# crockwell/rel_pose

Hardware: AMD Instinct MI355X
Metric: image-pairs/sec fwd+bwd @384x384, 1/2/4/8 MI355X; R,t err vs ref (higher is better)
Workload: dtype f32; 1 GPU; train.py step (ViTEss fwd + geodesic loss + bwd + grad all-reduce + clip + Adam), synthetic 384x384 pairs; scope=full, pairs_per_gpu=64, global_batch_pairs=64, parallelism=dp1, finite=True, gemm_operand_precision=exact fp32 MFMA, launch=eager

## Files before the change

__graft_entry__.py:

```python
import os
import subprocess
import sys

ROOT = os.path.dirname(os.path.abspath(__file__))
if ROOT not in sys.path:
    sys.path.insert(0, ROOT)


def build():
    import torch
    from rel_pose_amd import _build
    force = os.environ.get("RP_FORCE_BUILD", "" if torch.cuda.is_available() else "1") == "1"
    _build.build(force=force, verbose=True)
    from rel_pose_amd import _lib
    lib = _lib.load()
    assert lib.rp_abi_version() == _lib.ABI_VERSION and lib.rp_target_arch() == b"gfx950"
    assert lib.rp_abi_export_count() == _lib.ABI_EXPORTS == len(_lib.EXPORTS)
    assert _lib.load_readout().rp_readout_abi_version() == _lib.READOUT_ABI_VERSION
    assert _lib.load_eightpoint().rp_eightpoint_abi_version() == _lib.EIGHTPOINT_ABI_VERSION
    assert _lib.load_refine().rp_refine_abi_version() == _lib.REFINE_ABI_VERSION
    assert _lib.load_consensus().rp_consensus_abi_version() == _lib.CONSENSUS_ABI_VERSION
    assert _lib.load_submatch().rp_submatch_abi_version() == _lib.SUBMATCH_ABI_VERSION
    assert _lib.load_fivepoint().rp_fivepoint_abi_version() == _lib.FIVEPOINT_ABI_VERSION
    assert _lib.load_homography().rp_homography_abi_version() == _lib.HOMOGRAPHY_ABI_VERSION
    assert _lib.load_triangulate().rp_triangulate_abi_version() == _lib.TRIANGULATE_ABI_VERSION
    import rel_pose_amd.model
    import oracle.relpose_oracle
    print("build ok:", _lib.lib_path(), _build.READOUT_LIB, _build.EIGHTPOINT_LIB, _build.REFINE_LIB, _build.CONSENSUS_LIB, _build.SUBMATCH_LIB,
          _build.FIVEPOINT_LIB, _build.HOMOGRAPHY_LIB, _build.TRIANGULATE_LIB)


def smoke():
    import types

    import torch

    from oracle import relpose_oracle as O
    from rel_pose_amd import _lib
    from rel_pose_amd.model import ViTEss
    assert torch.cuda.is_available(), "smoke() needs cuda:0"
    _lib.load()
    torch.cuda.set_device(0)
    args = types.SimpleNamespace(noess="", pool_size=60, fc_hidden_size=512, fusion_transformer=True,
                                 transformer_depth=6, cross_features=False, use_single_softmax=False,
                                 no_pos_encoding=False, l1_pos_encoding=False)
    shapes = dict(O.vit_param_shapes())
    shapes.update(O.cnn_param_shapes())
    sd32, sd64 = O.make_state(shapes, torch.float32), O.make_state(shapes, torch.float64)
    model = ViTEss(args)
    model.load_state_dict(sd32)
    model = model.cuda().train()
    tok = O.synthetic_tokens(2)
    Gs = torch.tensor([0, 0, 0, 0, 0, 0, 1.0]).repeat(1, 2, 1)
    intr = torch.tensor([[30.0, 26.0, 12.0, 11.0]]).repeat(1, 2, 1)
    fmap = tok.permute(0, 2, 1).contiguous().view(2, 192, 24, 24).cuda().requires_grad_(True)
    out = model.forward_tokens(fmap, Gs.cuda(), intr.cuda())
    out[:, 1].square().sum().backward()
    t64 = tok.double().requires_grad_(True)
    ref = O.vit_ess_from_tokens(sd64, t64, Gs.double(), intr.double())
    ref[:, 1].square().sum().backward()
    t_err, q_err, ang = O.pose_errors(out.detach().cpu(), ref.detach())
    g_err = O.rel_err(fmap.grad.view(2, 192, 576).permute(0, 2, 1).cpu(), t64.grad)
    print("smoke: t_err=%.2e q_err=%.2e angle=%.2e rad, token-grad rel err=%.2e" % (t_err, q_err, ang, g_err))
    assert max(t_err, q_err) < 1e-4 and g_err < 2e-5
    print("smoke ok (HIP path vs CPU oracle)")


if __name__ == "__main__":
    build()
    if len(sys.argv) > 1 and sys.argv[1] == "smoke":
        smoke()
```

rel_pose_amd/_build.py:

```python
import os
import subprocess
import sys

HERE = os.path.dirname(os.path.abspath(__file__))
CSRC = os.path.join(HERE, "csrc")
LIB = os.path.join(HERE, "librelpose_hip.so")
SOURCES = ["gemm.hip", "gemm_dma.hip", "rowwise.hip", "attention.hip", "attention_bf16.hip", "dw192_bf16.hip", "dw192_f32.hip", "dw192_split3.hip", "dx_lnbwd_bf16.hip", "emm.hip", "emm_bf16.hip", "batchnorm.hip", "se3loss.hip", "geom.hip", "augment.hip", "mlp_fused.hip", "linear_rows.hip", "conv_stem.hip", "conv_stem_bf16.hip", "conv_stem_wgrad_bf16.hip", "conv_stem_wgrad_f32.hip", "conv3x3_bf16.hip", "conv3x3_wgrad_bf16.hip", "conv3x3_wgrad_f32.hip", "conv3x3_f32.hip", "conv3x3_c128_f32.hip"]
READOUT_CSRC = os.path.join(HERE, "csrc_readout")
READOUT_LIB = os.path.join(HERE, "librelpose_readout.so")
READOUT_SOURCES = ["emm_readout.hip"]
EIGHTPOINT_CSRC = os.path.join(HERE, "csrc_eightpoint")
EIGHTPOINT_LIB = os.path.join(HERE, "librelpose_eightpoint.so")
EIGHTPOINT_SOURCES = ["eight_point.hip"]
REFINE_CSRC = os.path.join(HERE, "csrc_refine")
REFINE_LIB = os.path.join(HERE, "librelpose_refine.so")
REFINE_SOURCES = ["refine_pose.hip"]
CONSENSUS_CSRC = os.path.join(HERE, "csrc_consensus")
CONSENSUS_LIB = os.path.join(HERE, "librelpose_consensus.so")
CONSENSUS_SOURCES = ["consensus.hip"]
SUBMATCH_CSRC = os.path.join(HERE, "csrc_submatch")
SUBMATCH_LIB = os.path.join(HERE, "librelpose_submatch.so")
SUBMATCH_SOURCES = ["submatch.hip"]
FIVEPOINT_CSRC = os.path.join(HERE, "csrc_fivepoint")
FIVEPOINT_LIB = os.path.join(HERE, "librelpose_fivepoint.so")
FIVEPOINT_SOURCES = ["five_point.hip"]
HOMOGRAPHY_CSRC = os.path.join(HERE, "csrc_homography")
HOMOGRAPHY_LIB = os.path.join(HERE, "librelpose_homography.so")
HOMOGRAPHY_SOURCES = ["homography.hip"]
TRIANGULATE_CSRC = os.path.join(HERE, "csrc_triangulate")
TRIANGULATE_LIB = os.path.join(HERE, "librelpose_triangulate.so")
TRIANGULATE_SOURCES = ["triangulate.hip"]
ARCH = "gfx950"


def _hipcc():
    for c in (os.environ.get("HIPCC"), "/opt/rocm/bin/hipcc"):
        if c and os.path.exists(c):
            return c
    return "hipcc"


def _stale(lib, csrc, sources, headers):
    if not os.path.exists(lib):
        return True
    t = os.path.getmtime(lib)
    return any(os.path.getmtime(d) > t for d in [os.path.join(csrc, s) for s in sources] + headers)


def needs_build():
    return _stale(LIB, CSRC, SOURCES, _headers())


def readout_needs_build():
    return _stale(READOUT_LIB, READOUT_CSRC, READOUT_SOURCES, _readout_headers())


def eightpoint_needs_build():
    return _stale(EIGHTPOINT_LIB, EIGHTPOINT_CSRC, EIGHTPOINT_SOURCES, _eightpoint_headers())


def refine_needs_build():
    return _stale(REFINE_LIB, REFINE_CSRC, REFINE_SOURCES, _refine_headers())


def consensus_needs_build():
    return _stale(CONSENSUS_LIB, CONSENSUS_CSRC, CONSENSUS_SOURCES, _consensus_headers())


def submatch_needs_build():
    return _stale(SUBMATCH_LIB, SUBMATCH_CSRC, SUBMATCH_SOURCES, _submatch_headers())


def fivepoint_needs_build():
    return _stale(FIVEPOINT_LIB, FIVEPOINT_CSRC, FIVEPOINT_SOURCES, _fivepoint_headers())


def homography_needs_build():
    return _stale(HOMOGRAPHY_LIB, HOMOGRAPHY_CSRC, HOMOGRAPHY_SOURCES, _homography_headers())


def triangulate_needs_build():
    return _stale(TRIANGULATE_LIB, TRIANGULATE_CSRC, TRIANGULATE_SOURCES, _triangulate_headers())


def build(force=False, verbose=True):
    import fcntl
    with open(os.path.join(HERE, ".build.lock"), "w") as lock:
        fcntl.flock(lock, fcntl.LOCK_EX)
        try:
            if force or needs_build():
                _build_locked(verbose, force, LIB, CSRC, SOURCES, _headers())
            if force or readout_needs_build():
                _build_locked(verbose, force, READOUT_LIB, READOUT_CSRC, READOUT_SOURCES, _readout_headers())
            if force or eightpoint_needs_build():
                _build_locked(verbose, force, EIGHTPOINT_LIB, EIGHTPOINT_CSRC, EIGHTPOINT_SOURCES, _eightpoint_headers())
            if force or refine_needs_build():
                _build_locked(verbose, force, REFINE_LIB, REFINE_CSRC, REFINE_SOURCES, _refine_headers())
            if force or consensus_needs_build():
                _build_locked(verbose, force, CONSENSUS_LIB, CONSENSUS_CSRC, CONSENSUS_SOURCES, _consensus_headers())
            if force or submatch_needs_build():
                _build_locked(verbose, force, SUBMATCH_LIB, SUBMATCH_CSRC, SUBMATCH_SOURCES, _submatch_headers())
            if force or fivepoint_needs_build():
                _build_locked(verbose, force, FIVEPOINT_LIB, FIVEPOINT_CSRC, FIVEPOINT_SOURCES, _fivepoint_headers())
            if force or homography_needs_build():
                _build_locked(verbose, force, HOMOGRAPHY_LIB, HOMOGRAPHY_CSRC, HOMOGRAPHY_SOURCES, _homography_headers())
            if force or triangulate_needs_build():
                _build_locked(verbose, force, TRIANGULATE_LIB, TRIANGULATE_CSRC, TRIANGULATE_SOURCES, _triangulate_headers())
            return LIB
        finally:
            fcntl.flock(lock, fcntl.LOCK_UN)


def _headers():
    return [os.path.join(CSRC, h) for h in sorted(os.listdir(CSRC)) if h.endswith(".h")] + \
           [os.path.join(os.path.dirname(HERE), "include", "relpose_hip.h")]


def _readout_headers():
    return _headers() + [os.path.join(os.path.dirname(HERE), "include", "relpose_readout.h")]


def _eightpoint_headers():
    return _headers() + [os.path.join(os.path.dirname(HERE), "include", "relpose_eightpoint.h")]


def _refine_headers():
    return _headers() + [os.path.join(os.path.dirname(HERE), "include", "relpose_refine.h")]


def _consensus_headers():
    return _headers() + [os.path.join(os.path.dirname(HERE), "include", "relpose_consensus.h")]


def _submatch_headers():
    return _headers() + [os.path.join(os.path.dirname(HERE), "include", "relpose_submatch.h")]


def _fivepoint_headers():
    return _headers() + [os.path.join(os.path.dirname(HERE), "include", "relpose_fivepoint.h")]


def _homography_headers():
    return _headers() + [os.path.join(os.path.dirname(HERE), "include", "relpose_homography.h")]


def _triangulate_headers():
    return _headers() + [os.path.join(os.path.dirname(HERE), "include", "relpose_triangulate.h")]


def _build_locked(verbose, force, lib, csrc, sources, headers):
    cc = _hipcc()
    objs = []
    procs = []
    hdr_t = max(os.path.getmtime(h) for h in headers)
    for s in sources:
        o = os.path.join(csrc, s.replace(".hip", ".o"))
        objs.append(o)
        if not force and os.path.exists(o) and os.path.getmtime(o) > max(hdr_t, os.path.getmtime(os.path.join(csrc, s))):
            continue
        cmd = [cc, "--offload-arch=" + ARCH, "-O3", "-std=c++17", "-fPIC", "-c", os.path.join(csrc, s), "-o", o]
        if verbose:
            print(" ".join(cmd), flush=True)
        procs.append((s, subprocess.Popen(cmd, stdout=subprocess.PIPE, stderr=subprocess.STDOUT)))
    for s, p in procs:
        out, _ = p.communicate()
        if p.returncode != 0:
            sys.stderr.write(out.decode())
            raise RuntimeError("hipcc failed on " + s)
    tmp = lib + ".tmp.%d" % os.getpid()
    cmd = [cc, "--offload-arch=" + ARCH, "-shared", "-fPIC", "-o", tmp] + objs
    if verbose:
        print(" ".join(cmd), flush=True)
    subprocess.check_call(cmd)
    os.replace(tmp, lib)
    return lib


if __name__ == "__main__":
    build(force="--force" in sys.argv)
```

rel_pose_amd/_lib.py:

```python
import ctypes
import keyword
import os
import re
from ctypes import POINTER, Structure, c_char_p, c_float, c_int, c_longlong, c_size_t, c_void_p

import torch

from . import _build

_LIB = None
HEADER = os.path.join(os.path.dirname(os.path.dirname(os.path.abspath(__file__))), "include", "relpose_hip.h")

_SCALARS = {"int": c_int, "float": c_float, "long long": c_longlong, "size_t": c_size_t}
_POINTEES = ("void", "float", "double", "int", "unsigned char")
_DEFINE = re.compile(r"#\s*define\s+(RP_\w+)\s+(-?\d+|\(-?\d+\))")
_DECL = re.compile(r"(const\s+)?(unsigned\s+char|long\s+long|\w+)\s*(\*?)\s*([A-Za-z_]\w*(?:\s*,\s*[A-Za-z_]\w*)*)?")
_ITEM = re.compile(r"\s*(?:typedef\s+struct\s+(\w+)\s*\{([^{}]*);\s*\}\s*(\w+)\s*;"
                   r"|([\w\s*]+?)\b(rp_\w+)\s*\(([^()]*)\)\s*;"
                   r'|extern\s+"C"\s*\{|\})')


def _declaration(text, structs, header="relpose_hip.h"):
    m = _DECL.fullmatch(text.strip())
    if not m:
# ... 54 lines not shown
with open(HEADER) as _f:
    _CONSTS, _STRUCTS, _PROTOTYPES, _STATUS = _header_contract(_f.read())
ABI_VERSION, ABI_EXPORTS = _CONSTS["RP_ABI_VERSION"], _CONSTS["RP_ABI_EXPORTS"]
RP_COLSUM_MAX, RP_SPLITK_MAX, RP_TRANSPOSE_MAX = _CONSTS["RP_COLSUM_MAX"], _CONSTS["RP_SPLITK_MAX"], _CONSTS["RP_TRANSPOSE_MAX"]
_ERROR_TEXT = {"RP_EBADSHAPE": "bad shape", "RP_EALIGN": "misaligned pointer/stride", "RP_EWORKSPACE": "workspace too small",
               "RP_EUNSUPPORTED": "unsupported"}
RP_ERRORS = {code: _ERROR_TEXT[name] for name, code in _CONSTS.items() if name.startswith("RP_E")}
RpGemm, RpColsumTask, RpBnMask, RpSplitkTask, RpTransposeTask = (
    _STRUCTS[n] for n in ("RpGemm", "RpColsumTask", "RpBnMask", "RpSplitkTask", "RpTransposeTask"))
EXPORTS = tuple(_PROTOTYPES)
DECLARED = set(EXPORTS)


_READOUT_LIB = None
READOUT_HEADER = os.path.join(os.path.dirname(HEADER), "relpose_readout.h")
with open(READOUT_HEADER) as _f:
    _READOUT_CONSTS, _, _READOUT_PROTOTYPES, _READOUT_STATUS = _header_contract(_f.read(), "relpose_readout.h")
READOUT_ABI_VERSION = _READOUT_CONSTS["RP_READOUT_ABI_VERSION"]
READOUT_EXPORTS = tuple(_READOUT_PROTOTYPES)


_EIGHTPOINT_LIB = None
EIGHTPOINT_HEADER = os.path.join(os.path.dirname(HEADER), "relpose_eightpoint.h")
with open(EIGHTPOINT_HEADER) as _f:
    _EIGHTPOINT_CONSTS, _, _EIGHTPOINT_PROTOTYPES, _EIGHTPOINT_STATUS = _header_contract(_f.read(), "relpose_eightpoint.h")
EIGHTPOINT_ABI_VERSION = _EIGHTPOINT_CONSTS["RP_EIGHTPOINT_ABI_VERSION"]
EIGHTPOINT_MAX_P, EIGHTPOINT_MAX_ITERS = _EIGHTPOINT_CONSTS["RP_EIGHTPOINT_MAX_P"], _EIGHTPOINT_CONSTS["RP_EIGHTPOINT_MAX_ITERS"]
EIGHTPOINT_EXPORTS = tuple(_EIGHTPOINT_PROTOTYPES)


_REFINE_LIB = None
REFINE_HEADER = os.path.join(os.path.dirname(HEADER), "relpose_refine.h")
with open(REFINE_HEADER) as _f:
    _REFINE_CONSTS, _, _REFINE_PROTOTYPES, _REFINE_STATUS = _header_contract(_f.read(), "relpose_refine.h")
REFINE_ABI_VERSION = _REFINE_CONSTS["RP_REFINE_ABI_VERSION"]
REFINE_MAX_P, REFINE_MAX_ITERS = _REFINE_CONSTS["RP_REFINE_MAX_P"], _REFINE_CONSTS["RP_REFINE_MAX_ITERS"]
REFINE_EXPORTS = tuple(_REFINE_PROTOTYPES)


_CONSENSUS_LIB = None
CONSENSUS_HEADER = os.path.join(os.path.dirname(HEADER), "relpose_consensus.h")
with open(CONSENSUS_HEADER) as _f:
    _CONSENSUS_CONSTS, _, _CONSENSUS_PROTOTYPES, _CONSENSUS_STATUS = _header_contract(_f.read(), "relpose_consensus.h")
CONSENSUS_ABI_VERSION = _CONSENSUS_CONSTS["RP_CONSENSUS_ABI_VERSION"]
CONSENSUS_MAX_P, CONSENSUS_MAX_M = _CONSENSUS_CONSTS["RP_CONSENSUS_MAX_P"], _CONSENSUS_CONSTS["RP_CONSENSUS_MAX_M"]
CONSENSUS_EXPORTS = tuple(_CONSENSUS_PROTOTYPES)


_SUBMATCH_LIB = None
SUBMATCH_HEADER = os.path.join(os.path.dirname(HEADER), "relpose_submatch.h")
with open(SUBMATCH_HEADER) as _f:
    _SUBMATCH_CONSTS, _, _SUBMATCH_PROTOTYPES, _SUBMATCH_STATUS = _header_contract(_f.read(), "relpose_submatch.h")
SUBMATCH_ABI_VERSION = _SUBMATCH_CONSTS["RP_SUBMATCH_ABI_VERSION"]
SUBMATCH_EXPORTS = tuple(_SUBMATCH_PROTOTYPES)


_FIVEPOINT_LIB = None
FIVEPOINT_HEADER = os.path.join(os.path.dirname(HEADER), "relpose_fivepoint.h")
with open(FIVEPOINT_HEADER) as _f:
    _FIVEPOINT_CONSTS, _, _FIVEPOINT_PROTOTYPES, _FIVEPOINT_STATUS = _header_contract(_f.read(), "relpose_fivepoint.h")
FIVEPOINT_ABI_VERSION = _FIVEPOINT_CONSTS["RP_FIVEPOINT_ABI_VERSION"]
FIVEPOINT_MAX_P, FIVEPOINT_MAX_M, FIVEPOINT_ROOTS = (_FIVEPOINT_CONSTS[k] for k in ("RP_FIVEPOINT_MAX_P", "RP_FIVEPOINT_MAX_M", "RP_FIVEPOINT_ROOTS"))
FIVEPOINT_EXPORTS = tuple(_FIVEPOINT_PROTOTYPES)


_HOMOGRAPHY_LIB = None
HOMOGRAPHY_HEADER = os.path.join(os.path.dirname(HEADER), "relpose_homography.h")
with open(HOMOGRAPHY_HEADER) as _f:
    _HOMOGRAPHY_CONSTS, _, _HOMOGRAPHY_PROTOTYPES, _HOMOGRAPHY_STATUS = _header_contract(_f.read(), "relpose_homography.h")
HOMOGRAPHY_ABI_VERSION = _HOMOGRAPHY_CONSTS["RP_HOMOGRAPHY_ABI_VERSION"]
HOMOGRAPHY_MAX_P, HOMOGRAPHY_MAX_M, HOMOGRAPHY_MAX_ITERS = (_HOMOGRAPHY_CONSTS[k] for k in ("RP_HOMOGRAPHY_MAX_P", "RP_HOMOGRAPHY_MAX_M", "RP_HOMOGRAPHY_MAX_ITERS"))
HOMOGRAPHY_EXPORTS = tuple(_HOMOGRAPHY_PROTOTYPES)


_TRIANGULATE_LIB = None
TRIANGULATE_HEADER = os.path.join(os.path.dirname(HEADER), "relpose_triangulate.h")
with open(TRIANGULATE_HEADER) as _f:
    _TRIANGULATE_CONSTS, _, _TRIANGULATE_PROTOTYPES, _TRIANGULATE_STATUS = _header_contract(_f.read(), "relpose_triangulate.h")
TRIANGULATE_ABI_VERSION = _TRIANGULATE_CONSTS["RP_TRIANGULATE_ABI_VERSION"]
TRIANGULATE_MAX_P = _TRIANGULATE_CONSTS["RP_TRIANGULATE_MAX_P"]
TRIANGULATE_EXPORTS = tuple(_TRIANGULATE_PROTOTYPES)


def lib_path():
    return _build.LIB


def load():
    global _LIB
    if _LIB is not None:
        return _LIB
    path = _build.LIB
    if _build.needs_build():
        _build.build(verbose=False)
    try:
        lib = ctypes.CDLL(path)
    except OSError as e:
        raise RuntimeError("rel_pose_amd: cannot load HIP extension %s (%s); there is no CPU fallback" % (path, e))
    lib.rp_abi_version.restype = c_int
    if lib.rp_abi_version() != ABI_VERSION:
        raise RuntimeError("rel_pose_amd: %s has ABI version %d, this package binds version %d -- rebuild with "
                           "`python -m rel_pose_amd._build --force`" % (path, lib.rp_abi_version(), ABI_VERSION))
    if len(EXPORTS) != ABI_EXPORTS:
        raise RuntimeError("rel_pose_amd: include/relpose_hip.h declares %d entry points (RP_ABI_EXPORTS = %d)" % (len(EXPORTS), ABI_EXPORTS))
    lib.rp_abi_export_count.restype = c_int
    if lib.rp_abi_export_count() != ABI_EXPORTS:
        raise RuntimeError("rel_pose_amd: %s was compiled with %d entry points, the header declares %d -- rebuild"
                           % (path, lib.rp_abi_export_count(), ABI_EXPORTS))
    for name, (res, args) in _PROTOTYPES.items():
        fn = getattr(lib, name)
        fn.restype = res
        fn.argtypes = args
        if name in _STATUS:
            fn.errcheck = _raise_on_status
    _LIB = lib
    return lib


def load_readout():
    global _READOUT_LIB
    if _READOUT_LIB is not None:
        return _READOUT_LIB
    path = _build.READOUT_LIB
    if _build.readout_needs_build():
        _build.build(verbose=False)
    try:
        lib = ctypes.CDLL(path)
    except OSError as e:
        raise RuntimeError("rel_pose_amd: cannot load HIP extension %s (%s); there is no CPU fallback" % (path, e))
    lib.rp_readout_abi_version.restype = c_int
    if lib.rp_readout_abi_version() != READOUT_ABI_VERSION:
        raise RuntimeError("rel_pose_amd: %s has ABI version %d, this package binds version %d -- rebuild with "
                           "`python -m rel_pose_amd._build --force`" % (path, lib.rp_readout_abi_version(), READOUT_ABI_VERSION))
    for name, (res, args) in _READOUT_PROTOTYPES.items():
        fn = getattr(lib, name)
        fn.restype = res
        fn.argtypes = args
        if name in _READOUT_STATUS:
            fn.errcheck = _raise_on_status
    _READOUT_LIB = lib
    return lib


def load_eightpoint():
    global _EIGHTPOINT_LIB
    if _EIGHTPOINT_LIB is not None:
        return _EIGHTPOINT_LIB
    path = _build.EIGHTPOINT_LIB
    if _build.eightpoint_needs_build():
        _build.build(verbose=False)
    try:
        lib = ctypes.CDLL(path)
    except OSError as e:
        raise RuntimeError("rel_pose_amd: cannot load HIP extension %s (%s); there is no CPU fallback" % (path, e))
    lib.rp_eightpoint_abi_version.restype = c_int
    if lib.rp_eightpoint_abi_version() != EIGHTPOINT_ABI_VERSION:
        raise RuntimeError("rel_pose_amd: %s has ABI version %d, this package binds version %d -- rebuild with "
                           "`python -m rel_pose_amd._build --force`" % (path, lib.rp_eightpoint_abi_version(), EIGHTPOINT_ABI_VERSION))
    for name, (res, args) in _EIGHTPOINT_PROTOTYPES.items():
        fn = getattr(lib, name)
        fn.restype = res
        fn.argtypes = args
        if name in _EIGHTPOINT_STATUS:
            fn.errcheck = _raise_on_status
    _EIGHTPOINT_LIB = lib
    return lib
# ... 69 lines not shown
        fn.restype = res
        fn.argtypes = args
        if name in _SUBMATCH_STATUS:
            fn.errcheck = _raise_on_status
    _SUBMATCH_LIB = lib
    return lib


def load_fivepoint():
    global _FIVEPOINT_LIB
    if _FIVEPOINT_LIB is not None:
        return _FIVEPOINT_LIB
    path = _build.FIVEPOINT_LIB
    if _build.fivepoint_needs_build():
        _build.build(verbose=False)
    try:
        lib = ctypes.CDLL(path)
    except OSError as e:
        raise RuntimeError("rel_pose_amd: cannot load HIP extension %s (%s); there is no CPU fallback" % (path, e))
    lib.rp_fivepoint_abi_version.restype = c_int
    if lib.rp_fivepoint_abi_version() != FIVEPOINT_ABI_VERSION:
        raise RuntimeError("rel_pose_amd: %s has ABI version %d, this package binds version %d -- rebuild with "
                           "`python -m rel_pose_amd._build --force`" % (path, lib.rp_fivepoint_abi_version(), FIVEPOINT_ABI_VERSION))
    for name, (res, args) in _FIVEPOINT_PROTOTYPES.items():
        fn = getattr(lib, name)
        fn.restype = res
        fn.argtypes = args
        if name in _FIVEPOINT_STATUS:
            fn.errcheck = _raise_on_status
    _FIVEPOINT_LIB = lib
    return lib


def load_homography():
    global _HOMOGRAPHY_LIB
    if _HOMOGRAPHY_LIB is not None:
        return _HOMOGRAPHY_LIB
    path = _build.HOMOGRAPHY_LIB
    if _build.homography_needs_build():
        _build.build(verbose=False)
    try:
        lib = ctypes.CDLL(path)
    except OSError as e:
        raise RuntimeError("rel_pose_amd: cannot load HIP extension %s (%s); there is no CPU fallback" % (path, e))
    lib.rp_homography_abi_version.restype = c_int
    if lib.rp_homography_abi_version() != HOMOGRAPHY_ABI_VERSION:
        raise RuntimeError("rel_pose_amd: %s has ABI version %d, this package binds version %d -- rebuild with "
                           "`python -m rel_pose_amd._build --force`" % (path, lib.rp_homography_abi_version(), HOMOGRAPHY_ABI_VERSION))
    for name, (res, args) in _HOMOGRAPHY_PROTOTYPES.items():
        fn = getattr(lib, name)
        fn.restype = res
        fn.argtypes = args
        if name in _HOMOGRAPHY_STATUS:
            fn.errcheck = _raise_on_status
    _HOMOGRAPHY_LIB = lib
    return lib


def load_triangulate():
    global _TRIANGULATE_LIB
    if _TRIANGULATE_LIB is not None:
        return _TRIANGULATE_LIB
    path = _build.TRIANGULATE_LIB
    if _build.triangulate_needs_build():
        _build.build(verbose=False)
    try:
        lib = ctypes.CDLL(path)
    except OSError as e:
        raise RuntimeError("rel_pose_amd: cannot load HIP extension %s (%s); there is no CPU fallback" % (path, e))
    lib.rp_triangulate_abi_version.restype = c_int
    if lib.rp_triangulate_abi_version() != TRIANGULATE_ABI_VERSION:
        raise RuntimeError("rel_pose_amd: %s has ABI version %d, this package binds version %d -- rebuild with "
                           "`python -m rel_pose_amd._build --force`" % (path, lib.rp_triangulate_abi_version(), TRIANGULATE_ABI_VERSION))
    for name, (res, args) in _TRIANGULATE_PROTOTYPES.items():
        fn = getattr(lib, name)
        fn.restype = res
        fn.argtypes = args
        if name in _TRIANGULATE_STATUS:
            fn.errcheck = _raise_on_status
    _TRIANGULATE_LIB = lib
    return lib


def _raise_on_status(rc, func, args):
    check(rc, func.__name__)
    return rc


def check(rc, what):
    if rc != 0:
        if rc < 0:
            raise RuntimeError("rel_pose_amd: %s failed: %s (RP error %d)" % (what, RP_ERRORS.get(rc, "?"), rc))
        raise RuntimeError("rel_pose_amd: %s failed: hipError %d" % (what, rc))
```

rel_pose_amd/ops.py:

```python
import ctypes
import itertools
import math
import os
import threading

import torch

from . import _lib

N_TOK = 576
DIM = 192
HEADS = 3
LN_EPS = 1e-6
XW = 96
GW = 224
NWG = 6


def _chk(*ts):
    for t in ts:
        if t is None:
            continue
        if not (t.is_cuda and t.dtype == torch.float32 and t.is_contiguous()):
            raise RuntimeError("rel_pose_amd ops need contiguous fp32 GPU tensors (no CPU fallback exists); got "
# ... 1774 lines not shown
                                    want_stats=bn is not None, bn=None if bn is None else bn[1:])
                if bn is not None:
                    if len(_BN_PENDING) > 64:
                        _BN_PENDING.clear()
                    _BN_PENDING[bn[0]] = (r[0].data_ptr(), r[1])
                    r = r[0]
                dx = r.permute(0, 3, 1, 2)
            else:
                dx = torch.ops.aten.convolution_backward(dy, x, w, None, [1, 1], [1, 1], [1, 1], False, [0, 0], 1, [True, False, False])[0]
                if dshared is not None:
                    dx = dx + dshared
        if ctx.needs_input_grad[1]:
            if CONV3X3_WGRAD_F32 and x.shape[0] >= CONV3X3_WGRAD_F32_MIN_N:
                dw = conv3x3_c64_wgrad_f32(_nhwc(x), dy.permute(0, 2, 3, 1)).permute(0, 3, 1, 2)
            else:
                dw = torch.ops.aten.convolution_backward(dy, x, w, None, [1, 1], [1, 1], [1, 1], False, [0, 0], 1, [False, True, False])[1]
        return dx, dw, None, None, None


CONV3X3_C128_F32 = os.environ.get("RP_CONV3X3_C128_F32", "1") != "0"
CONV_F32_STATS = os.environ.get("RP_CONV_F32_STATS", "1") != "0"
CONV3X3_C128_F32_MIN_N = int(os.environ.get("RP_CONV3X3_C128_F32_MIN_N", "56"))


def conv3x3_c128_f32(x_nhwc, w_ohwi, bias=None, input_gradient=False, want_stats=False):
    lib = _lib.load()
    if not (x_nhwc.is_cuda and x_nhwc.is_contiguous() and x_nhwc.dtype == torch.float32 and tuple(x_nhwc.shape[1:]) == (28, 28, 128)):
        raise RuntimeError("conv3x3_c128_f32: contiguous fp32 [N,28,28,128] GPU tensor expected")
    CO = w_ohwi.shape[0]
    if not (w_ohwi.is_cuda and w_ohwi.is_contiguous() and w_ohwi.dtype == torch.float32 and tuple(w_ohwi.shape[1:]) == (3, 3, 128)
            and CO in (128, 192)):
        raise RuntimeError("conv3x3_c128_f32: contiguous fp32 [128 | 192,3,3,128] GPU filter expected")
    if input_gradient and (CO != 128 or bias is not None):
        raise RuntimeError("conv3x3_c128_f32: the input gradient needs the square 128 -> 128 filter and takes no bias")
    if bias is not None and not (bias.is_cuda and bias.is_contiguous() and bias.dtype == torch.float32 and tuple(bias.shape) == (CO,)):
        raise RuntimeError("conv3x3_c128_f32: contiguous fp32 [CO] GPU bias expected")
    N = x_nhwc.shape[0]
    y = torch.empty(N, 28, 28, CO, device=x_nhwc.device, dtype=torch.float32)
    stats = (torch.empty(lib.rp_conv3x3_c128_f32_blocks(N, CO) // (CO // 64), 2, CO, device=x_nhwc.device, dtype=torch.float64)
             if want_stats else None)
    with timed("conv3x3_c128_f32", 2.0 * N * 28 * 28 * 128 * CO * 9, 4.0 * N * 28 * 28 * (128 + CO)):
        lib.rp_conv3x3_c128_f32(_p(x_nhwc), _p(w_ohwi), _p(bias), _p(y), _p(stats), N, 28, 28, CO, 1 if input_gradient else 0,
                                _st())
    return (y, stats) if want_stats else y


class Conv3x3C128F32Fn(_Fn):

    @staticmethod
    def forward(ctx, x, w, bias, want_stats=False):
        ctx.save_for_backward(x, w)
        ctx.has_bias = bias is not None
        if want_stats and CONV_F32_STATS:
            y, stats = conv3x3_c128_f32(_nhwc(x), _nhwc(w), bias, want_stats=True)
            ctx.mark_non_differentiable(stats)
            return y.permute(0, 3, 1, 2), stats
        y = conv3x3_c128_f32(_nhwc(x), _nhwc(w), bias).permute(0, 3, 1, 2)
        return (y, None) if want_stats else y

    @staticmethod
    def backward(ctx, dy, *_):
        x, w = ctx.saved_tensors
        dx = dw = db = None
        dy = dy.contiguous(memory_format=torch.channels_last)
        CO = w.shape[0]
        own_dx = ctx.needs_input_grad[0] and CO == 128
        if own_dx:
            dx = conv3x3_c128_f32(_nhwc(dy), _nhwc(w), input_gradient=True).permute(0, 3, 1, 2)
        mask = [bool(ctx.needs_input_grad[0]) and not own_dx, bool(ctx.needs_input_grad[1]), ctx.has_bias and bool(ctx.needs_input_grad[2])]
        if any(mask):
            g = torch.ops.aten.convolution_backward(dy, x, w, [CO] if ctx.has_bias else None, [1, 1], [1, 1], [1, 1], False, [0, 0], 1, mask)
            dx = g[0] if mask[0] else dx
            dw = g[1] if mask[1] else None
            db = g[2] if mask[2] else None
        return dx, dw, db, None


def conv3x3_c128_f32_ok(m, x):
    return (CONV3X3_C128_F32 and CNN_PRECISION == 0 and x.is_cuda and x.dtype == torch.float32 and tuple(m.weight.shape[1:]) == (128, 3, 3)
            and m.weight.shape[0] in (128, 192) and m.stride == (1, 1) and m.padding == (1, 1) and m.dilation == (1, 1) and m.groups == 1
            and getattr(m, "padding_mode", "zeros") == "zeros" and tuple(x.shape[1:]) == (128, 28, 28) and x.shape[0] >= CONV3X3_C128_F32_MIN_N)


def conv3x3_wgrad_f32_ok(m, x):
    return (CONV3X3_WGRAD_F32 and CNN_PRECISION == 0 and x.is_cuda and x.dtype == torch.float32 and torch.is_grad_enabled()
            and m.weight.requires_grad and tuple(m.weight.shape) == (64, 64, 3, 3) and m.bias is None and m.stride == (1, 1)
            and m.padding == (1, 1) and m.dilation == (1, 1) and m.groups == 1 and tuple(x.shape[1:]) == (64, 56, 56)
            and x.shape[0] >= CONV3X3_WGRAD_F32_MIN_N)


def conv3x3_f32_ok(m, x):
    return (CONV3X3_F32 and CNN_PRECISION == 0 and x.is_cuda and x.dtype == torch.float32 and tuple(m.weight.shape) == (64, 64, 3, 3)
            and m.bias is None and m.stride == (1, 1) and m.padding == (1, 1) and m.dilation == (1, 1) and m.groups == 1
            and tuple(x.shape[1:]) == (64, 56, 56) and x.shape[0] >= CONV3X3_F32_MIN_N)


def conv3x3_own_ok(m, x):
    return (CONV3X3_OWN and CNN_PRECISION == 1 and x.is_cuda and tuple(m.weight.shape) == (64, 64, 3, 3) and m.bias is None
            and m.stride == (1, 1) and m.padding == (1, 1) and m.dilation == (1, 1) and m.groups == 1 and tuple(x.shape[1:]) == (64, 56, 56))


def conv2d(m, x, want_stats=False):
    if want_stats:
        if conv3x3_own_ok(m, x) and getattr(m, "_rp_bf16", None) is not None:
            xb = x if x.dtype == torch.bfloat16 else x.to(torch.bfloat16)
            return Conv3x3C64Fn.apply(xb, m._rp_bf16[0], True)
        if CNN_PRECISION == 0 and x.is_cuda and torch.is_grad_enabled():
            bn_src = getattr(x, "_rp_bn", None) if CONV_F32_BN_BWD else None
            if conv3x3_f32_ok(m, x):
                return Conv3x3C64F32Fn.apply(x, m.weight, True, False, bn_src)
            if conv3x3_c128_f32_ok(m, x):
                return Conv3x3C128F32Fn.apply(x, m.weight, m.bias, True)
        return conv2d(m, x), None
    if CNN_PRECISION == 0 or not x.is_cuda:
        if conv3x3_wgrad_f32_ok(m, x) or conv3x3_f32_ok(m, x):
            return Conv3x3C64F32Fn.apply(x, m.weight, False, False, None)
        if conv3x3_c128_f32_ok(m, x):
            return Conv3x3C128F32Fn.apply(x, m.weight, m.bias, False)
        return m(x)
    bf = torch.bfloat16
    ready = getattr(m, "_rp_bf16", None)
    if ready is not None and conv3x3_own_ok(m, x):
        return Conv3x3C64Fn.apply(x if x.dtype == bf else x.to(bf), ready[0], False)
    if ready is not None:
        xb = x if x.dtype == bf else x.to(bf)
        if (m.stride == (1, 1) and m.dilation == (1, 1) and m.groups == 1 and m.kernel_size[0] == m.kernel_size[1]
                and m.kernel_size[0] >= CONV_BWD_AS_FWD_MIN_K):
            return ConvBf16Fn.apply(xb, ready[0], ready[1], m.padding)
        return torch.nn.functional.conv2d(xb, ready[0], ready[1], m.stride, m.padding, m.dilation, m.groups)
    return torch.nn.functional.conv2d(x if x.dtype == bf else x.to(bf), m.weight.to(bf), None if m.bias is None else m.bias.to(bf),
                                      m.stride, m.padding, m.dilation, m.groups)


CONV_F32_SHARE_INPUT = os.environ.get("RP_CONV_F32_SHARE_INPUT", "1") != "0"


def conv2d_shared(m, x):
    if (CONV_F32_SHARE_INPUT and CNN_PRECISION == 0 and x.is_cuda and torch.is_grad_enabled() and x.requires_grad):
        if conv3x3_f32_ok(m, x):
            return Conv3x3C64F32Fn.apply(x, m.weight, True, True, None)
    y, st = conv2d(m, x, want_stats=True)
    return y, st, x


_NBT_PENDING = None


class batches_tracked_batch:

    def __enter__(self):
        global _NBT_PENDING
        self.prev, _NBT_PENDING = _NBT_PENDING, []
        return self

    def __exit__(self, et, ev, tb):
        global _NBT_PENDING
        cur, _NBT_PENDING = _NBT_PENDING, self.prev
        if et is None and cur:
            torch._foreach_add_(cur, 1)
        return False


def _bump_batches_tracked(bn):
    if _NBT_PENDING is not None and bn.num_batches_tracked is not None:
        _NBT_PENDING.append(bn.num_batches_tracked)
    else:
        bn.num_batches_tracked += 1


def bn_act(bn, x, residual=None, relu=True, stats=None):
    if not x.is_cuda:
        y = bn(x)
        if residual is not None:
            y = y + residual
        return torch.relu(y) if relu else y
    if bn.training and bn.track_running_stats:
        _bump_batches_tracked(bn)
    y = BnActFn.apply(x, bn.weight, bn.bias, bn.running_mean, bn.running_var, residual, bn.training, bn.momentum, bn.eps,
                      relu, stats if bn.training else None)
    if _BN_LAST is not None:
        y._rp_bn = _BN_LAST
    return y


class GeodesicLossFn(_Fn):

    @staticmethod
    def forward(ctx, Ps, Gs):
        lib = _lib.load()
        Ps, Gs = Ps.contiguous(), Gs.contiguous()
        _chk(Ps, Gs)
        B = Gs.shape[0]
        losses = _empty(2, like=Gs)
        dmean = _empty(2, B, 2, 7, like=Gs)
        scratch = _empty(60 * B, like=Gs)
        lib.rp_geodesic_loss(_p(Ps), _p(Gs), _p(losses), _p(dmean), _p(scratch), B, _st())
        ctx.save_for_backward(dmean)
        return losses[0], losses[1]

    @staticmethod
    def backward(ctx, gtr, grot):
# ... 298 lines not shown
```

Baseline: 1994 image-pairs/sec.

## Add custom fp32 MFMA dgrad kernel for 5x5 valid conv

Adds a new HIP library with an fp32 MFMA kernel that computes the input gradient of the 5x5 stride-1 valid convolution (192 output channels, 28x28 input) in NHWC. It tiles 128 images per block at each output pixel, orders pixels by tap count, and double-buffers dy and weight tiles via direct global-to-LDS loads. A new autograd function routes the backward input gradient through this kernel and keeps aten for the weight and bias gradients. This replaces the generic library convolution backward, at the cost of extra channels-last layout conversions and a strict batch-size gate.

Measured after the change: 2019 image-pairs/sec (median of 6 runs). 1.01x the previous value.

```diff
diff --git a/__graft_entry__.py b/__graft_entry__.py
--- a/__graft_entry__.py
+++ b/__graft_entry__.py
@@ -24,10 +24,11 @@
     assert _lib.load_fivepoint().rp_fivepoint_abi_version() == _lib.FIVEPOINT_ABI_VERSION
     assert _lib.load_homography().rp_homography_abi_version() == _lib.HOMOGRAPHY_ABI_VERSION
     assert _lib.load_triangulate().rp_triangulate_abi_version() == _lib.TRIANGULATE_ABI_VERSION
+    assert _lib.load_conv5x5().rp_conv5x5_abi_version() == _lib.CONV5X5_ABI_VERSION
     import rel_pose_amd.model
     import oracle.relpose_oracle
     print("build ok:", _lib.lib_path(), _build.READOUT_LIB, _build.EIGHTPOINT_LIB, _build.REFINE_LIB, _build.CONSENSUS_LIB, _build.SUBMATCH_LIB,
-          _build.FIVEPOINT_LIB, _build.HOMOGRAPHY_LIB, _build.TRIANGULATE_LIB)
+          _build.FIVEPOINT_LIB, _build.HOMOGRAPHY_LIB, _build.TRIANGULATE_LIB, _build.CONV5X5_LIB)
 
 
 def smoke():
diff --git a/include/relpose_conv5x5.h b/include/relpose_conv5x5.h
--- /dev/null
+++ b/include/relpose_conv5x5.h
@@ -0,0 +1,18 @@
+#ifndef RELPOSE_CONV5X5_H
+#define RELPOSE_CONV5X5_H
+
+#include "relpose_hip.h"
+
+#ifdef __cplusplus
+extern "C" {
+#endif
+
+#define RP_CONV5X5_ABI_VERSION 1
+int rp_conv5x5_abi_version(void);
+
+int rp_conv5x5_dgrad_f32(const float* dy, const float* w, float* dx, int N, int CI, const float* res, void* stream);
+
+#ifdef __cplusplus
+}
+#endif
+#endif
diff --git a/rel_pose_amd/_build.py b/rel_pose_amd/_build.py
--- a/rel_pose_amd/_build.py
+++ b/rel_pose_amd/_build.py
@@ -30,6 +30,9 @@
 TRIANGULATE_CSRC = os.path.join(HERE, "csrc_triangulate")
 TRIANGULATE_LIB = os.path.join(HERE, "librelpose_triangulate.so")
 TRIANGULATE_SOURCES = ["triangulate.hip"]
+CONV5X5_CSRC = os.path.join(HERE, "csrc_conv5x5")
+CONV5X5_LIB = os.path.join(HERE, "librelpose_conv5x5.so")
+CONV5X5_SOURCES = ["conv5x5_dgrad_f32.hip"]
 ARCH = "gfx950"
 
 
@@ -83,6 +86,10 @@
     return _stale(TRIANGULATE_LIB, TRIANGULATE_CSRC, TRIANGULATE_SOURCES, _triangulate_headers())
 
 
+def conv5x5_needs_build():
+    return _stale(CONV5X5_LIB, CONV5X5_CSRC, CONV5X5_SOURCES, _conv5x5_headers())
+
+
 def build(force=False, verbose=True):
     import fcntl
     with open(os.path.join(HERE, ".build.lock"), "w") as lock:
@@ -106,6 +113,8 @@
                 _build_locked(verbose, force, HOMOGRAPHY_LIB, HOMOGRAPHY_CSRC, HOMOGRAPHY_SOURCES, _homography_headers())
             if force or triangulate_needs_build():
                 _build_locked(verbose, force, TRIANGULATE_LIB, TRIANGULATE_CSRC, TRIANGULATE_SOURCES, _triangulate_headers())
+            if force or conv5x5_needs_build():
+                _build_locked(verbose, force, CONV5X5_LIB, CONV5X5_CSRC, CONV5X5_SOURCES, _conv5x5_headers())
             return LIB
         finally:
             fcntl.flock(lock, fcntl.LOCK_UN)
@@ -148,6 +157,10 @@
     return _headers() + [os.path.join(os.path.dirname(HERE), "include", "relpose_triangulate.h")]
 
 
+def _conv5x5_headers():
+    return _headers() + [os.path.join(os.path.dirname(HERE), "include", "relpose_conv5x5.h")]
+
+
 def _build_locked(verbose, force, lib, csrc, sources, headers):
     cc = _hipcc()
     objs = []
diff --git a/rel_pose_amd/_lib.py b/rel_pose_amd/_lib.py
--- a/rel_pose_amd/_lib.py
+++ b/rel_pose_amd/_lib.py
@@ -160,6 +160,14 @@
 TRIANGULATE_EXPORTS = tuple(_TRIANGULATE_PROTOTYPES)
 
 
+_CONV5X5_LIB = None
+CONV5X5_HEADER = os.path.join(os.path.dirname(HEADER), "relpose_conv5x5.h")
+with open(CONV5X5_HEADER) as _f:
+    _CONV5X5_CONSTS, _, _CONV5X5_PROTOTYPES, _CONV5X5_STATUS = _header_contract(_f.read(), "relpose_conv5x5.h")
+CONV5X5_ABI_VERSION = _CONV5X5_CONSTS["RP_CONV5X5_ABI_VERSION"]
+CONV5X5_EXPORTS = tuple(_CONV5X5_PROTOTYPES)
+
+
 def lib_path():
     return _build.LIB
 
@@ -395,6 +403,31 @@
     return lib
 
 
+def load_conv5x5():
+    global _CONV5X5_LIB
+    if _CONV5X5_LIB is not None:
+        return _CONV5X5_LIB
+    path = _build.CONV5X5_LIB
+    if _build.conv5x5_needs_build():
+        _build.build(verbose=False)
+    try:
+        lib = ctypes.CDLL(path)
+    except OSError as e:
+        raise RuntimeError("rel_pose_amd: cannot load HIP extension %s (%s); there is no CPU fallback" % (path, e))
+    lib.rp_conv5x5_abi_version.restype = c_int
+    if lib.rp_conv5x5_abi_version() != CONV5X5_ABI_VERSION:
+        raise RuntimeError("rel_pose_amd: %s has ABI version %d, this package binds version %d -- rebuild with "
+                           "`python -m rel_pose_amd._build --force`" % (path, lib.rp_conv5x5_abi_version(), CONV5X5_ABI_VERSION))
+    for name, (res, args) in _CONV5X5_PROTOTYPES.items():
+        fn = getattr(lib, name)
+        fn.restype = res
+        fn.argtypes = args
+        if name in _CONV5X5_STATUS:
+            fn.errcheck = _raise_on_status
+    _CONV5X5_LIB = lib
+    return lib
+
+
 def _raise_on_status(rc, func, args):
     check(rc, func.__name__)
     return rc
diff --git a/rel_pose_amd/csrc_conv5x5/conv5x5_dgrad_f32.hip b/rel_pose_amd/csrc_conv5x5/conv5x5_dgrad_f32.hip
--- /dev/null
+++ b/rel_pose_amd/csrc_conv5x5/conv5x5_dgrad_f32.hip
@@ -0,0 +1,210 @@
+#include "../csrc/common.h"
+#include "../../include/relpose_conv5x5.h"
+
+namespace {
+
+constexpr int CO = 192;
+constexpr int HO = 24;
+constexpr int HI = 28;
+constexpr int KS = 5;
+constexpr int PIX = HI * HI;
+constexpr int IB = 128;
+constexpr int SK = 64;
+constexpr int FOLD = 5;
+constexpr int A_FL = IB * SK;
+constexpr int DY_IMG = HO * HO * CO;
+
+constexpr int tap_lo(int v) { return v > HO - 1 ? v - (HO - 1) : 0; }
+constexpr int tap_hi(int v) { return v < KS - 1 ? v : KS - 1; }
+constexpr int taps(int pix) {
+  const int y = pix / HI, x = pix % HI;
+  return (tap_hi(y) - tap_lo(y) + 1) * (tap_hi(x) - tap_lo(x) + 1);
+}
+
+struct Order { unsigned short v[PIX]; };
+constexpr Order make_order() {
+  Order o{};
+  int k = 0;
+  for (int t = KS * KS; t >= 1; --t)
+    for (int p = 0; p < PIX; ++p)
+      if (taps(p) == t) o.v[k++] = (unsigned short)p;
+  Order q = o;
+  for (int j = 0; j < 400; ++j) q.v[j] = o.v[50 * (j & 7) + (j >> 3)];
+  return q;
+}
+__constant__ Order ORDER = make_order();
+
+struct Dg {
+  const float* dy; const float* w; const float* res; float* dx;
+  int N, groups;
+};
+
+template <int CI>
+__global__ __launch_bounds__(256, 1) void conv5x5_dgrad_f32_kernel(Dg p) {
+  constexpr int B_FL = SK * CI;
+  constexpr int CB = CI / 64;
+  constexpr int NA = A_FL / 1024;
+  constexpr int NB = B_FL / 1024;
+  constexpr int KSTEPS = SK / 2;
+  static_assert(NA + NB <= KSTEPS, "one DMA piece per k-step");
+  __shared__ __attribute__((aligned(16))) float As[2][A_FL];
+  __shared__ __attribute__((aligned(16))) float Bs[2][B_FL];
+  const int tid = threadIdx.x, lane = tid & 63, wave = __builtin_amdgcn_readfirstlane(tid >> 6), l31 = lane & 31, hi = lane >> 5;
+  const int pos = blockIdx.x / p.groups, grp = blockIdx.x - pos * p.groups;
+  const int pix = ORDER.v[pos], y = pix / HI, x = pix - y * HI;
+  const int r0 = tap_lo(y), r1 = tap_hi(y), s0 = tap_lo(x), s1 = tap_hi(x);
+  const int nst = (CO / SK) * (r1 - r0 + 1) * (s1 - s0 + 1);
+  const int n0 = grp * IB;
+  const float* dyb = p.dy + (long long)n0 * DY_IMG;
+
+  unsigned aoff[NA], boff[NB];
+#pragma unroll
+  for (int i = 0; i < NA; ++i) {
+    const int row = 4 * (wave + 4 * i) + (lane >> 4);
+    const int img = min(row, p.N - 1 - n0);
+    aoff[i] = (unsigned)img * (unsigned)(DY_IMG * 4) + (unsigned)((((lane & 15) ^ (row & 15))) << 4);
+  }
+#pragma unroll
+  for (int i = 0; i < NB; ++i) {
+    const int byte = (wave + 4 * i) * 1024 + lane * 16;
+    const int row = byte / (CI * 4), c = byte % (CI * 4);
+    boff[i] = (unsigned)(row * (KS * KS * CI * 4) + c);
+  }
+  const unsigned as0 = lds_byte_addr(&As[0][0]) + wave * 1024, bs0 = lds_byte_addr(&Bs[0][0]) + wave * 1024;
+  auto a_src = [&](int ch, int r, int s) { return uniform_ptr(dyb + ((y - r) * HO + (x - s)) * CO + ch * SK); };
+  auto b_src = [&](int ch, int r, int s) { return uniform_ptr(p.w + ((long long)(ch * SK) * (KS * KS) + r * KS + s) * CI); };
+
+  const int wr = wave >> 1, wc = wave & 1;
+  const int m15 = l31 & 15;
+  const int ao = (64 * wr + l31) * (SK / 4);
+  const int bo = 4 * hi * CI + (CI / 2) * wc + l31;
+  f32x16 acc[2][CB], sum[2][CB];
+#pragma unroll
+  for (int b = 0; b < 2; ++b)
+#pragma unroll
+    for (int j = 0; j < CB; ++j) acc[b][j] = sum[b][j] = zero16();
+  int fold = FOLD;
+
+  int nch = 0, nr = r0, ns = s0;
+  {
+    const void* sa = a_src(nch, nr, ns);
+    const void* sb = b_src(nch, nr, ns);
+#pragma unroll
+    for (int i = 0; i < NA; ++i) glds16(sa, aoff[i], as0 + i * 4096);
+#pragma unroll
+    for (int i = 0; i < NB; ++i) glds16(sb, boff[i], bs0 + i * 4096);
+  }
+  asm volatile("s_waitcnt vmcnt(0)" ::: "memory");
+  __builtin_amdgcn_s_barrier();
+  for (int st = 0; st < nst; ++st) {
+    const int buf = st & 1;
+    if (st + 1 < nst) {
+      if (ns < s1) ++ns;
+      else {
+        ns = s0;
+        if (nr < r1) ++nr;
+        else { nr = r0; ++nch; }
+      }
+    }
+    const void* sa = a_src(nch, nr, ns);
+    const void* sb = b_src(nch, nr, ns);
+    const unsigned an0 = as0 + (buf ^ 1) * (A_FL * 4), bn0 = bs0 + (buf ^ 1) * (B_FL * 4);
+    const float4* ap = reinterpret_cast<const float4*>(As[buf]) + ao;
+    const unsigned bt = lds_byte_addr(Bs[buf] + bo);
+    float4 ac[2], an[2];
+    float bf[CB], bn[CB];
+#pragma unroll
+    for (int b = 0; b < 2; ++b) ac[b] = ap[b * 32 * (SK / 4) + (hi ^ m15)];
+    static_for<CB>([&](auto j) { bf[j] = lds_rd32<128 * j>(bt); });
+    static_for<KSTEPS>([&](auto tt) {
+      constexpr int t = tt, g = t / 4, e = t % 4;
+      if constexpr (CB == 3) asm volatile("s_waitcnt lgkmcnt(0)" : "+v"(bf[0]), "+v"(bf[1]), "+v"(bf[CB - 1]));
+      else asm volatile("s_waitcnt lgkmcnt(0)" : "+v"(bf[0]), "+v"(bf[1]));
+      if constexpr (t + 1 < KSTEPS) {
+        constexpr int g1 = (t + 1) / 4, e1 = (t + 1) % 4;
+        static_for<CB>([&](auto j) { bn[j] = lds_rd32<((8 * g1 + e1) * CI + 32 * j) * 4>(bt); });
+        if constexpr (e == 0 && g + 1 < KSTEPS / 4) {
+#pragma unroll
+          for (int b = 0; b < 2; ++b) an[b] = ap[b * 32 * (SK / 4) + ((2 * (g + 1) + hi) ^ m15)];
+        }
+      }
+      if constexpr (t < NA) glds16(sa, aoff[t < NA ? t : 0], an0 + t * 4096);
+      else if constexpr (t < NA + NB) glds16(sb, boff[t >= NA && t < NA + NB ? t - NA : 0], bn0 + (t - NA) * 4096);
+      __builtin_amdgcn_sched_barrier(0);
+#pragma unroll
+      for (int b = 0; b < 2; ++b) {
+        const float av = e == 0 ? ac[b].x : e == 1 ? ac[b].y : e == 2 ? ac[b].z : ac[b].w;
+#pragma unroll
+        for (int j = 0; j < CB; ++j) acc[b][j] = mfma32(av, bf[j], acc[b][j]);
+      }
+      if constexpr (t + 1 < KSTEPS) {
+#pragma unroll
+        for (int j = 0; j < CB; ++j) bf[j] = bn[j];
+        if constexpr (e == 3) {
+          ac[0] = an[0];
+          ac[1] = an[1];
+        }
+      }
+      __builtin_amdgcn_sched_barrier(0);
+    });
+    if (--fold == 0) {
+      fold = FOLD;
+#pragma unroll
+      for (int b = 0; b < 2; ++b)
+#pragma unroll
+        for (int j = 0; j < CB; ++j) {
+          sum[b][j] += acc[b][j];
+          acc[b][j] = zero16();
+        }
+    }
+    asm volatile("s_waitcnt vmcnt(0) lgkmcnt(0)" ::: "memory");
+    __builtin_amdgcn_s_barrier();
+  }
+#pragma unroll
+  for (int b = 0; b < 2; ++b)
+#pragma unroll
+    for (int j = 0; j < CB; ++j) acc[b][j] += sum[b][j];
+
+  const int ci = (CI / 2) * wc + l31;
+  const float* __restrict__ res = p.res;
+  float* __restrict__ dx = p.dx;
+#pragma unroll
+  for (int b = 0; b < 2; ++b) {
+    const int img0 = n0 + 64 * wr + 32 * b;
+    if (res) {
+#pragma unroll
+      for (int r = 0; r < 16; ++r) {
+        const size_t o = ((size_t)min(img0 + acc_row(r, hi), p.N - 1) * PIX + pix) * CI + ci;
+#pragma unroll
+        for (int j = 0; j < CB; ++j) acc[b][j][r] += res[o + 32 * j];
+      }
+    }
+#pragma unroll
+    for (int r = 0; r < 16; ++r) {
+      const int img = img0 + acc_row(r, hi);
+      if (img < p.N) {
+        const size_t o = ((size_t)img * PIX + pix) * CI + ci;
+#pragma unroll
+        for (int j = 0; j < CB; ++j) dx[o + 32 * j] = acc[b][j][r];
+      }
+    }
+  }
+}
+
+}
+
+extern "C" int rp_conv5x5_abi_version(void) { return RP_CONV5X5_ABI_VERSION; }
+
+extern "C" int rp_conv5x5_dgrad_f32(const float* dy, const float* w, float* dx, int N, int CI, const float* res, void* stream) {
+  if (N < 1 || !dy || !w || !dx) return RP_EBADSHAPE;
+  if (CI != 128 && CI != 192) return RP_EUNSUPPORTED;
+  if (((uintptr_t)dy | (uintptr_t)w | (uintptr_t)dx | (uintptr_t)res) & 15) return RP_EALIGN;
+  Dg p;
+  p.dy = dy; p.w = w; p.res = res; p.dx = dx; p.N = N;
+  p.groups = (N + IB - 1) / IB;
+  const dim3 grid((unsigned)PIX * (unsigned)p.groups);
+  if (CI == 192) hipLaunchKernelGGL(conv5x5_dgrad_f32_kernel<192>, grid, dim3(256), 0, (hipStream_t)stream, p);
+  else hipLaunchKernelGGL(conv5x5_dgrad_f32_kernel<128>, grid, dim3(256), 0, (hipStream_t)stream, p);
+  RP_CHECK_LAUNCH();
+  return RP_OK;
+}
diff --git a/rel_pose_amd/ops.py b/rel_pose_amd/ops.py
--- a/rel_pose_amd/ops.py
+++ b/rel_pose_amd/ops.py
@@ -1880,6 +1880,61 @@
             and getattr(m, "padding_mode", "zeros") == "zeros" and tuple(x.shape[1:]) == (128, 28, 28) and x.shape[0] >= CONV3X3_C128_F32_MIN_N)
 
 
+CONV5X5_DGRAD_F32 = os.environ.get("RP_CONV5X5_DGRAD_F32", "1") != "0"
+CONV5X5_DGRAD_F32_MIN_N = int(os.environ.get("RP_CONV5X5_DGRAD_F32_MIN_N", "112"))
+CONV5X5_DGRAD_IMAGES = 128
+
+
+def conv5x5_dgrad_f32(dy_nhwc, w_ohwi, res_nhwc=None):
+    lib = _lib.load_conv5x5()
+    if not (dy_nhwc.is_cuda and dy_nhwc.is_contiguous() and dy_nhwc.dtype == torch.float32 and dy_nhwc.dim() == 4
+            and tuple(dy_nhwc.shape[1:]) == (24, 24, 192) and dy_nhwc.shape[0] >= 1):
+        raise RuntimeError("conv5x5_dgrad_f32: contiguous fp32 [N,24,24,192] GPU tensor expected")
+    CI = w_ohwi.shape[-1]
+    if not (w_ohwi.is_cuda and w_ohwi.is_contiguous() and w_ohwi.dtype == torch.float32 and tuple(w_ohwi.shape[:3]) == (192, 5, 5)
+            and CI in (128, 192)):
+        raise RuntimeError("conv5x5_dgrad_f32: contiguous fp32 [192,5,5,128 | 192] GPU filter expected")
+    N = dy_nhwc.shape[0]
+    if res_nhwc is not None and not (res_nhwc.is_cuda and res_nhwc.is_contiguous() and res_nhwc.dtype == torch.float32
+                                     and tuple(res_nhwc.shape) == (N, 28, 28, CI)):
+        raise RuntimeError("conv5x5_dgrad_f32: contiguous fp32 [N,28,28,CI] GPU residual expected")
+    dx = torch.empty(N, 28, 28, CI, device=dy_nhwc.device, dtype=torch.float32)
+    lib.rp_conv5x5_dgrad_f32(_p(dy_nhwc), _p(w_ohwi), _p(dx), N, CI, _p(res_nhwc), _st())
+    return dx
+
+
+class Conv5x5ValidF32Fn(_Fn):
+
+    @staticmethod
+    def forward(ctx, x, w, bias):
+        ctx.save_for_backward(x, w)
+        ctx.has_bias = bias is not None
+        return torch.nn.functional.conv2d(x, w, bias)
+
+    @staticmethod
+    def backward(ctx, dy):
+        x, w = ctx.saved_tensors
+        dx = dw = db = None
+        dy = dy.contiguous(memory_format=torch.channels_last)
+        if ctx.needs_input_grad[0]:
+            dx = conv5x5_dgrad_f32(_nhwc(dy), _nhwc(w)).permute(0, 3, 1, 2)
+        mask = [False, bool(ctx.needs_input_grad[1]), ctx.has_bias and bool(ctx.needs_input_grad[2])]
+        if any(mask):
+            g = torch.ops.aten.convolution_backward(dy, x, w, [192] if ctx.has_bias else None, [1, 1], [0, 0], [1, 1], False, [0, 0], 1, mask)
+            dw = g[1] if mask[1] else None
+            db = g[2] if mask[2] else None
+        return dx, dw, db
+
+
+def conv5x5_dgrad_f32_ok(m, x):
+    n = x.shape[0]
+    return (CONV5X5_DGRAD_F32 and CNN_PRECISION == 0 and x.is_cuda and x.dtype == torch.float32 and torch.is_grad_enabled()
+            and x.requires_grad and tuple(m.kernel_size) == (5, 5) and m.stride == (1, 1) and m.padding == (0, 0) and m.dilation == (1, 1)
+            and m.groups == 1 and m.weight.shape[0] == 192 and tuple(x.shape[1:]) in ((192, 28, 28), (128, 28, 28))
+            and tuple(m.weight.shape[1:]) == (x.shape[1], 5, 5) and n >= CONV5X5_DGRAD_F32_MIN_N
+            and (n - 1) % CONV5X5_DGRAD_IMAGES + 1 >= CONV5X5_DGRAD_F32_MIN_N)
+
+
 def conv3x3_wgrad_f32_ok(m, x):
     return (CONV3X3_WGRAD_F32 and CNN_PRECISION == 0 and x.is_cuda and x.dtype == torch.float32 and torch.is_grad_enabled()
             and m.weight.requires_grad and tuple(m.weight.shape) == (64, 64, 3, 3) and m.bias is None and m.stride == (1, 1)
@@ -1915,6 +1970,8 @@
             return Conv3x3C64F32Fn.apply(x, m.weight, False, False, None)
         if conv3x3_c128_f32_ok(m, x):
             return Conv3x3C128F32Fn.apply(x, m.weight, m.bias, False)
+        if conv5x5_dgrad_f32_ok(m, x):
+            return Conv5x5ValidF32Fn.apply(x, m.weight, m.bias)
         return m(x)
     bf = torch.bfloat16
     ready = getattr(m, "_rp_bf16", None)
```
